# geopti/mjlab-1

Hardware: AMD Instinct MI355X
Metric: env-steps/sec, Unitree-G1 velocity task num_envs=4096, 1/2/4/8 MI355X (higher is better)
Workload: dtype f32

## Files before the change

mjlab-1_amd/csrc/engine_impl.h:

```cpp
#pragma once
#include <float.h>
#include <stdlib.h>
#include <algorithm>
#include <initializer_list>
#include <utility>
#include <math.h>

#include "engine.h"

#pragma clang fp contract(on)

namespace mjx {

#define MINVAL 1e-15f
#define MINMU 1e-5f
#define MINIMP 0.0001f
#define MAXIMP 0.9999f


struct V3 { float x, y, z; };
__device__ __forceinline__ V3 v3(const float* p) { return {p[0], p[1], p[2]}; }
__device__ __forceinline__ void st3(float* p, V3 a) { p[0] = a.x; p[1] = a.y; p[2] = a.z; }
__device__ __forceinline__ V3 operator+(V3 a, V3 b) { return {a.x + b.x, a.y + b.y, a.z + b.z}; }
__device__ __forceinline__ V3 operator-(V3 a, V3 b) { return {a.x - b.x, a.y - b.y, a.z - b.z}; }
// ... 2059 lines not shown
      spd_factor_solve_tree<NR, SP>(S + L.M, S + L.H, S + L.qacc_smooth, S + L.chol, nvp, lane);
    else
      spd_factor_solve<NR>(S + L.M, nullptr, S + L.H, S + L.qacc_smooth, S + L.chol, nvp, lane);
    const float qacs_i = lane < nvq ? S[L.qacc_smooth + lane] : 0.f;
    if (lane < nvq) gw[LB.qacc_smooth + lane] = qacs_i;
    STAMP(7);
    if (obs) {
      float* mb = S + L.crb;
      if (bl) mb[B.b] = B.mass;
      sync();
      const V3 X = v3(S + L.subtree_com + 3 * B.b);
      const V3 vown = v3(S + L.stlin + 3 * B.b);
      V3 pv = {0.f, 0.f, 0.f}, hs = {0.f, 0.f, 0.f}, cx = {0.f, 0.f, 0.f}, mr = {0.f, 0.f, 0.f};
#pragma unroll 4
      for (int c = 0; c < nb; c++) {
        const bool in = (B.sub >> c) & 1ull;
        const float f = in ? mb[c] : 0.f, fh = in ? 1.f : 0.f;
        const V3 r = v3(S + L.xipos + 3 * c) - X;
        const V3 vc = v3(S + L.stlin + 3 * c);
        pv = pv + vc * f;
        hs = hs + v3(S + L.stang + 3 * c) * fh;
        cx = cx + cross(r, vc) * f;
        mr = mr + r * f;
      }
      sync();
      if (bl) {
        const float sm = stm;
        const V3 V = sm > MINVAL ? pv * (1.0f / sm) : vown;
        st3(S + L.stlin + 3 * B.b, V);
        st3(S + L.stang + 3 * B.b, hs + cx - cross(mr, V));
      }
      sync();
    }
    for (int s = lane; obs && s < d.nsensor; s += kWave) {
      if (m.sensor_type[s] != SENS_SUBTREEANGMOM) continue;
      float* out = D.sensordata + (size_t)w * d.nsensordata + m.sensor_adr[s];
      const int obj = m.sensor_objid[s];
      out[0] = S[L.stang + 3 * obj]; out[1] = S[L.stang + 3 * obj + 1]; out[2] = S[L.stang + 3 * obj + 2];
    }
    if (last) {
      const size_t wb = (size_t)w * nb;
      for (int i = lane; i < 3 * nb; i += kWave) {
        D.subtree_linvel[wb * 3 + i] = S[L.stlin + i];
        D.subtree_angmom[wb * 3 + i] = S[L.stang + i];
      }
    }
    sync();
    STAMP(8);
    if (lane == 0) { ints[0] = 0; ints[1] = 0; ints[2] = 0; ints[3] = 0; }
    {
      const float* gpos = MF(geom_pos);
      const float* gquat = MF(geom_quat);
      for (int sl = lane; sl < d.ngeom_lds; sl += kWave) {
        const int g = m.lds_geom[sl];
        int b = m.geom_bodyid[g];
        const Q4 qb = q4(S + L.xquat + 4 * b);
        st3(S + L.gxpos + 3 * sl, v3(S + L.xpos + 3 * b) + qrot(qb, v3(gpos + 3 * g)));
        qmat(S + L.gxmat + 9 * sl, qmul(qb, q4(gquat + 4 * g)));
      }
    }
    sync();
    {
      ConOut co{S, ints, &L, d.nconmax};
      const float* gsize = MF(geom_size);
      const float* grb = MF(geom_rbound);
      const float* gmargin = MF(geom_margin);
      const bool rec = m.pair_rec != nullptr && m.geom_rbound_ws == 0 && m.geom_margin_ws == 0;
      for (int p = lane; p < d.npair; p += kWave) {
        int g1, g2, t1, t2, l1, l2;
        float margin, cull;
        if (rec) {
          const int4 rc = reinterpret_cast<const int4*>(m.pair_rec)[p];
          g1 = rc.x & 0xffff; g2 = (int)((unsigned)rc.x >> 16);
          l1 = rc.y & 0xfff; l2 = (rc.y >> 12) & 0xfff;
          t1 = (rc.y >> 24) & 15; t2 = (int)((unsigned)rc.y >> 28);
          margin = __int_as_float(rc.z);
          cull = __int_as_float(rc.w);
        } else {
          g1 = m.pair_geom1[p]; g2 = m.pair_geom2[p];
          t1 = m.geom_type[g1]; t2 = m.geom_type[g2];
          l1 = m.geom_lds[g1]; l2 = m.geom_lds[g2];
          margin = fmaxf(gmargin[g1], gmargin[g2]);
          const float r1 = grb[g1], r2 = grb[g2];
          cull = (r1 > 0 && r2 > 0 && t1 != GEOM_HFIELD) ? r1 + r2 + margin : INFINITY;
        }
        V3 p1 = v3(S + L.gxpos + 3 * l1), p2 = v3(S + L.gxpos + 3 * l2);
        if (norm(p2 - p1) > cull) continue;
        const float* s1 = gsize + 3 * g1;
        const float* s2 = gsize + 3 * g2;
        int key = p * 8;
        if (t1 == GEOM_PLANE) {
          const float* Rp = S + L.gxmat + 9 * l1;
          V3 n = {Rp[2], Rp[5], Rp[8]};
          if (t2 == GEOM_SPHERE) {
            plane_sphere(co, key, g1, g2, p1, n, p2, s2[0], margin);
          } else if (t2 == GEOM_CAPSULE) {
            const float* R2 = S + L.gxmat + 9 * l2;
            V3 ax = {R2[2], R2[5], R2[8]};
            int k = key;
            k += plane_sphere(co, k, g1, g2, p1, n, p2 + ax * s2[1], s2[0], margin);
            plane_sphere(co, k, g1, g2, p1, n, p2 - ax * s2[1], s2[0], margin);
          } else if (t2 == GEOM_BOX) {
            float dist = dot(p2 - p1, n);
            const float* R2 = S + L.gxmat + 9 * l2;
            int cnt = 0;
            for (int i = 0; i < 8 && cnt < 4; i++) {
              V3 v = {(i & 1) ? s2[0] : -s2[0], (i & 2) ? s2[1] : -s2[1], (i & 4) ? s2[2] : -s2[2]};
              V3 corner = mulv(R2, v);
              float ld = dot(n, corner);
              if (dist + ld > margin || ld > 0) continue;
              append(co, key + cnt, g1, g2, dist + ld, corner + p2 - n * (0.5f * (dist + ld)), n);
              cnt++;
            }
          } else {
            atomicOr(&ints[3], 4);
          }
        } else if (t1 == GEOM_SPHERE && t2 == GEOM_SPHERE) {
          sphere_sphere(co, key, g1, g2, p1, s1[0], p2, s2[0], margin);
        } else if (t1 == GEOM_SPHERE && t2 == GEOM_CAPSULE) {
          const float* R2 = S + L.gxmat + 9 * l2;
          V3 ax = {R2[2], R2[5], R2[8]};
          V3 pa, pb;
          seg_seg(p1, p1, p2 + ax * s2[1], p2 - ax * s2[1], &pa, &pb);
          sphere_sphere(co, key, g1, g2, p1, s1[0], pb, s2[0], margin);
        } else if (t1 == GEOM_CAPSULE && t2 == GEOM_CAPSULE) {
          const float* R1 = S + L.gxmat + 9 * l1;
          const float* R2 = S + L.gxmat + 9 * l2;
          const V3 a1 = {R1[2], R1[5], R1[8]}, a2 = {R2[2], R2[5], R2[8]};
          capsule_capsule(co, key, g1, g2, p1, a1 * s1[1], s1[0], p2, a2 * s2[1], s2[0], margin);
        } else if (t1 == GEOM_BOX && t2 == GEOM_BOX) {
          HFrame F1, F2;
          F1.p = p1; F2.p = p2;
          for (int i = 0; i < 9; i++) { F1.R[i] = S[L.gxmat + 9 * l1 + i]; F2.R[i] = S[L.gxmat + 9 * l2 + i]; }
          if constexpr (kBoxBox<SP>) box_box(co, key, g1, g2, F1, v3(s1), F2, v3(s2), margin);
        } else if (t2 == GEOM_BOX && (t1 == GEOM_SPHERE || t1 == GEOM_CAPSULE)) {
          HFrame F;
          F.p = p2;
#pragma unroll
          for (int i = 0; i < 9; i++) F.R[i] = S[L.gxmat + 9 * l2 + i];
          if (t1 == GEOM_SPHERE) {
            box_sphere(co, key, g1, g2, F, v3(s2), mulTv(F.R, p1 - F.p), s1[0], margin);
          } else {
            const float* R1 = S + L.gxmat + 9 * l1;
            box_capsule(co, key, g1, g2, F, v3(s2), p1, V3{R1[2], R1[5], R1[8]}, s1[1], s1[0], margin);
          }
        } else {
          atomicOr(&ints[3], 4);
        }
      }
      if (d.nstatic > 0) {
        float lo0 = 1e30f, lo1 = 1e30f, lo2 = 1e30f, hi0 = -1e30f, hi1 = -1e30f, hi2 = -1e30f;
        for (int i = lane; i < d.nstpartner; i += kWave) {
          const int g = m.st_partner[i];
          const V3 c = v3(S + L.gxpos + 3 * m.geom_lds[g]);
          const float r = grb[g] + gmargin[g];
          lo0 = fminf(lo0, c.x - r); lo1 = fminf(lo1, c.y - r); lo2 = fminf(lo2, c.z - r);
          hi0 = fmaxf(hi0, c.x + r); hi1 = fmaxf(hi1, c.y + r); hi2 = fmaxf(hi2, c.z + r);
        }
        lo0 = wave_min(lo0); lo1 = wave_min(lo1); lo2 = wave_min(lo2);
        hi0 = wave_max(hi0); hi1 = wave_max(hi1); hi2 = wave_max(hi2);
        auto overlap = [&](const float* bb) {
          return bb[0] <= hi0 && bb[3] >= lo0 && bb[1] <= hi1 && bb[4] >= lo1 && bb[2] <= hi2 &&
                 bb[5] >= lo2;
        };
        const float* gpos = MF(geom_pos);
        const float* gquat = MF(geom_quat);
        const float* hsz_all = MF(hfield_size);
        const float* hdat_all = MF(hfield_data);
        int trunc = 0;
        static_assert(kStaticChunk == kWave, "lane per terrain geom of a chunk");
        const int nchunk = (d.nstatic + kStaticChunk - 1) / kStaticChunk;
        for (int cb = 0; cb < nchunk; cb += kWave) {
          const int c = cb + lane;
          unsigned long long cbal = __ballot(c < nchunk && overlap(m.st_chunk_aabb + 6 * c));
          while (cbal) {
            const int ch = cb + __ffsll((long long)cbal) - 1;
            cbal &= cbal - 1;
            const int i = ch * kStaticChunk + lane;
            unsigned long long bal = __ballot(i < d.nstatic && overlap(m.st_aabb + 6 * i));
            while (bal) {
              const int j = ch * kStaticChunk + __ffsll((long long)bal) - 1;
              bal &= bal - 1;
              const int sg = m.st_geom[j];
              const HFrame F = hfield_frame(m, S, L, gpos, gquat, sg);
              if (m.geom_type[sg] == GEOM_HFIELD) {
                const int hid = m.geom_dataid[sg];
                const float* hs = hsz_all + 4 * hid;
                const float* hd = hdat_all + m.hfield_adr[hid];
                const int nr = m.hfield_nrow[hid], nc = m.hfield_ncol[hid];
                for (int p = m.st_pairadr[j] + lane; p < m.st_pairadr[j + 1]; p += kWave) {
                  const int g2 = m.pair_geom2[p];
                  const int t2 = m.geom_type[g2];
                  const int l2 = m.geom_lds[g2];
                  const V3 p2 = v3(S + L.gxpos + 3 * l2);
                  const float* s2 = gsize + 3 * g2;
                  const float margin = fmaxf(gmargin[sg], gmargin[g2]);
                  const int key = p * 8;
                  if (t2 == GEOM_SPHERE) {
                    hfield_sphere(co, key, sg, g2, F, hd, hs, nr, nc, p2, s2[0], margin, &trunc);
                  } else if (t2 == GEOM_CAPSULE) {
                    const float* R2 = S + L.gxmat + 9 * l2;
                    const V3 ax = {R2[2], R2[5], R2[8]};
                    int k = key;
                    k += hfield_sphere(co, k, sg, g2, F, hd, hs, nr, nc, p2 + ax * s2[1], s2[0], margin, &trunc);
                    hfield_sphere(co, k, sg, g2, F, hd, hs, nr, nc, p2 - ax * s2[1], s2[0], margin, &trunc);
                  } else {
                    atomicOr(&ints[3], 4);
                  }
                }
              } else {
                const float* bb = m.st_aabb + 6 * j;
                const V3 bs = v3(gsize + 3 * sg);
                for (int p = m.st_pairadr[j] + lane; p < m.st_pairadr[j + 1]; p += kWave) {
                  const int pa = m.pair_geom1[p], pb = m.pair_geom2[p];
                  const int g1 = pa == sg ? pb : pa;
                  const int t1 = m.geom_type[g1];
                  const int l1 = m.geom_lds[g1];
                  const V3 p1 = v3(S + L.gxpos + 3 * l1);
                  const float margin = fmaxf(gmargin[sg], gmargin[g1]);
                  const float rr = grb[g1] + margin;
                  if (p1.x + rr < bb[0] || p1.x - rr > bb[3] || p1.y + rr < bb[1] ||
                      p1.y - rr > bb[4] || p1.z + rr < bb[2] || p1.z - rr > bb[5]) continue;
                  const float* s1 = gsize + 3 * g1;
                  const int key = p * 8;
                  if (t1 == GEOM_SPHERE) {
                    box_sphere(co, key, g1, sg, F, bs, mulTv(F.R, p1 - F.p), s1[0], margin);
                  } else if (t1 == GEOM_CAPSULE) {
                    const float* R1 = S + L.gxmat + 9 * l1;
                    box_capsule(co, key, g1, sg, F, bs, p1, V3{R1[2], R1[5], R1[8]}, s1[1], s1[0], margin);
                  } else if (t1 == GEOM_BOX) {
                    HFrame Fp;
                    Fp.p = p1;
                    for (int i = 0; i < 9; i++) Fp.R[i] = S[L.gxmat + 9 * l1 + i];
                    if constexpr (kBoxBox<SP>) {
                      if (pa == sg) box_box(co, key, pa, pb, F, bs, Fp, v3(s1), margin);
                      else box_box(co, key, pa, pb, Fp, v3(s1), F, bs, margin);
                    }
                  } else {
                    atomicOr(&ints[3], 4);
                  }
                }
              }
            }
          }
        }
        if (trunc) atomicOr(&ints[3], 4);
      }
    }
    sync();
    STAMP(3);
    int ncon = min(ints[0], d.nconmax);
    {
      auto contact_params = [&](int c, int g1, int g2, float dist) {
        const float* fri = MF(geom_friction);
        const float* sref = MF(geom_solref);
        const float* simp = MF(geom_solimp);
        const float* smix = MF(geom_solmix);
        const float* gmar = MF(geom_margin);
        const float* ggap = MF(geom_gap);
        int p1 = m.geom_priority[g1], p2 = m.geom_priority[g2];
        int dim;
        float f0, f1;
        float sr[2], si[5];
        if (p1 != p2) {
          int g = p1 > p2 ? g1 : g2;
          dim = m.geom_condim[g];
          f0 = fri[3 * g]; f1 = fri[3 * g + 1];
          sr[0] = sref[2 * g]; sr[1] = sref[2 * g + 1];
          for (int i = 0; i < 5; i++) si[i] = simp[5 * g + i];
        } else {
          dim = max(m.geom_condim[g1], m.geom_condim[g2]);
          f0 = fmaxf(fri[3 * g1], fri[3 * g2]);
          f1 = fmaxf(fri[3 * g1 + 1], fri[3 * g2 + 1]);
          float s1 = smix[g1], s2 = smix[g2], mix;
          if (s1 < MINVAL && s2 < MINVAL) mix = 0.5f;
          else if (s1 < MINVAL) mix = 0.f;
          else if (s2 < MINVAL) mix = 1.f;
          else mix = s1 / (s1 + s2);
          const float* r1 = sref + 2 * g1;
          const float* r2 = sref + 2 * g2;
          if (r1[0] > 0 && r2[0] > 0) {
            sr[0] = mix * r1[0] + (1 - mix) * r2[0];
            sr[1] = mix * r1[1] + (1 - mix) * r2[1];
          } else {
            sr[0] = fminf(r1[0], r2[0]);
            sr[1] = fminf(r1[1], r2[1]);
          }
          for (int i = 0; i < 5; i++) si[i] = mix * simp[5 * g1 + i] + (1 - mix) * simp[5 * g2 + i];
        }
        (void)f1;
        S[L.con_mu + 2 * c] = fmaxf(MINMU, f0);
        S[L.con_mu + 2 * c + 1] = fmaxf(MINMU, f0);
        Si[L.con_dim + c] = dim;
        const float imargin = fmaxf(gmar[g1], gmar[g2]) - fmaxf(ggap[g1], ggap[g2]);
        S[L.con_imargin + c] = imargin;
        S[L.con_imp + c] = impedance(si, dist, imargin);
        solref_kb(sr, si, h, S[L.con_kb + 2 * c], S[L.con_kb + 2 * c + 1]);
      };
      auto con_bodies = [&](int g1, int g2) {
        const int b1 = m.geom_bodyid[g1], b2 = m.geom_bodyid[g2];
        return b1 | b2 << 8 | m.body_rootid[b1] << 16 | m.body_rootid[b2] << 24;
      };
      if (kCon1<SP> || ncon <= kWave) {
        int key = lane < ncon ? Si[L.con_key + lane] : 0x7fffffff;
        int idx = lane;
#pragma unroll
        for (int k = 2; k <= kWave; k <<= 1) {
#pragma unroll
          for (int j = k >> 1; j > 0; j >>= 1) {
            int pk = __shfl_xor(key, j);
            int pi = __shfl_xor(idx, j);
            bool up = (lane & k) == 0;
            bool lower = (lane & j) == 0;
            bool sw = lower ? (up ? key > pk : key < pk) : (up ? key < pk : key > pk);
            if (sw) { key = pk; idx = pi; }
          }
        }
        int g1 = 0, g2 = 0;
        float dist = 0, px = 0, py = 0, pz = 0, nx = 0, ny = 0, nz = 0;
        if (lane < ncon) {
          g1 = Si[L.con_g1 + idx]; g2 = Si[L.con_g2 + idx]; dist = S[L.con_dist + idx];
          px = S[L.con_pos + 3 * idx]; py = S[L.con_pos + 3 * idx + 1]; pz = S[L.con_pos + 3 * idx + 2];
          nx = S[L.con_n + 3 * idx]; ny = S[L.con_n + 3 * idx + 1]; nz = S[L.con_n + 3 * idx + 2];
        }
        sync();
        if (lane < ncon) {
          Si[L.con_g1 + lane] = g1; Si[L.con_g2 + lane] = g2; S[L.con_dist + lane] = dist;
          Si[L.con_key + lane] = con_bodies(g1, g2);
          S[L.con_pos + 3 * lane] = px; S[L.con_pos + 3 * lane + 1] = py; S[L.con_pos + 3 * lane + 2] = pz;
          V3 n = {nx, ny, nz};
          n = n * (1.0f / fmaxf(norm(n), MINVAL));
          st3(S + L.con_n + 3 * lane, n);
          contact_params(lane, g1, g2, dist);
        }
      } else if constexpr (!kCon1<SP>) {
        int* perm = Si + L.efc_cid;
        const int rounds = (ncon + kWave - 1) / kWave;
        for (int c = lane; c < ncon; c += kWave) {
          const int kc = Si[L.con_key + c];
          int rank = 0;
          for (int j = 0; j < ncon; j++) rank += Si[L.con_key + j] < kc ? 1 : 0;
          perm[rank] = c;
        }
        sync();
        auto permute = [&](float* base, int stride, int comp) {
          float v[kMaxConRounds];
#pragma unroll
          for (int r = 0; r < kMaxConRounds; r++) {
            const int c = lane + r * kWave;
            v[r] = r < rounds && c < ncon ? base[stride * perm[c] + comp] : 0.f;
          }
          sync();
#pragma unroll
          for (int r = 0; r < kMaxConRounds; r++) {
            const int c = lane + r * kWave;
            if (r < rounds && c < ncon) base[stride * c + comp] = v[r];
          }
          sync();
        };
        permute(reinterpret_cast<float*>(Si + L.con_g1), 1, 0);
        permute(reinterpret_cast<float*>(Si + L.con_g2), 1, 0);
        permute(S + L.con_dist, 1, 0);
        for (int t = 0; t < 3; t++) permute(S + L.con_pos, 3, t);
        for (int t = 0; t < 3; t++) permute(S + L.con_n, 3, t);
        for (int c = lane; c < ncon; c += kWave) {
          const int g1 = Si[L.con_g1 + c], g2 = Si[L.con_g2 + c];
          Si[L.con_key + c] = con_bodies(g1, g2);
          V3 n = v3(S + L.con_n + 3 * c);
          n = n * (1.0f / fmaxf(norm(n), MINVAL));
          st3(S + L.con_n + 3 * c, n);
          contact_params(c, g1, g2, S[L.con_dist + c]);
        }
      }
      sync();
    }
    STAMP(4);
    {
      const float* jrange = MF(jnt_range);
      const float* jmargin = MF(jnt_margin);
      int nlim_rows = 0;
      int lim_mask = 0;
      if (lane < d.njnt && m.jnt_limited[lane] &&
          (m.jnt_type[lane] == JNT_HINGE || m.jnt_type[lane] == JNT_SLIDE)) {
        float q = S[L.qpos + m.jnt_qposadr[lane]];
        float mg = jmargin[lane];
        if (q - jrange[2 * lane] < mg) lim_mask |= 1;
        if (jrange[2 * lane + 1] - q < mg) lim_mask |= 2;
        nlim_rows = (lim_mask & 1) + ((lim_mask >> 1) & 1);
      }
      int lim_total, lim_off = wave_excl_scan(nlim_rows, lane, &lim_total);
      const bool con1 = kCon1<SP> || ncon <= kWave;
      int cdim = 0, crow = 0, con_total = 0, con_off = 0;
      if (con1) {
        cdim = lane < ncon ? Si[L.con_dim + lane] : 0;
        crow = lane < ncon ? (cdim == 1 ? 1 : 2 * (cdim - 1)) : 0;
        if (lane < ncon && cdim != 1 && cdim != 3) atomicOr(&ints[3], 4);
        con_off = wave_excl_scan(crow, lane, &con_total);
      } else {
        for (int c0 = 0; c0 < ncon; c0 += kWave) {
          const int c = c0 + lane;
          const int cd = c < ncon ? Si[L.con_dim + c] : 0;
          const int cr = c < ncon ? (cd == 1 ? 1 : 2 * (cd - 1)) : 0;
          if (c < ncon && cd != 1 && cd != 3) atomicOr(&ints[3], 4);
          int tot, off = wave_excl_scan(cr, lane, &tot);
          if (c < ncon) Si[L.con_efc + c] = con_total + off;
          con_total += tot;
        }
      }
      auto con_rows = [&](int c) {
        const int cd = Si[L.con_dim + c];
        return cd == 1 ? 1 : 2 * (cd - 1);
      };
      int nefc = lim_total + con_total;
      if (P->ovf_resolve) {
        const bool over = ints[0] > d.nconmax || nefc > d.njmax;
        int slot = -1;
        if (over && lane == 0) {
          const int li = 2 * split + ((sel_arg & kSelAPar) ? 1 : 0);
          slot = atomicAdd(P->ovf_n + li, 1);
          if (slot < P->ovf_cap) {
            P->ovf_list[(size_t)li * P->ovf_cap + slot] = w;
            atomicAdd(D.evtotal + 3, 1);
          }
        }
        slot = __shfl(slot, 0);
        const bool listed = over && slot < P->ovf_cap;
        if (lane == 0) {
          P->ovf_flag[w] = listed ? 1 : 0;
          if (listed) D.nefc[w] = -1;
        }
        if (listed) return;
      }
      if (nefc > d.njmax) {
        if (lane == 0) atomicOr(&ints[3], 2);
      }
      int keep_con = ncon;
      if (con1) {
        bool fits = lane < ncon && lim_total + con_off + crow <= d.njmax;
        unsigned long long bal = __ballot(lane < ncon && !fits);
        if (bal) keep_con = __ffsll((long long)bal) - 1;
        keep_con = min(keep_con, ncon);
        ncon = keep_con;
        nefc = lim_total + (ncon > 0 ? __shfl(con_off + crow, ncon - 1) : 0);
      } else {
        for (int c0 = 0; c0 < ncon; c0 += kWave) {
          const int c = c0 + lane;
          const bool fits = c < ncon && lim_total + Si[L.con_efc + c] + con_rows(c) <= d.njmax;
          const unsigned long long bal = __ballot(c < ncon && !fits);
          if (bal) { keep_con = c0 + __ffsll((long long)bal) - 1; break; }
        }
        ncon = keep_con;
        nefc = lim_total + (ncon > 0 ? Si[L.con_efc + ncon - 1] + con_rows(ncon - 1) : 0);
      }
      if (lim_total > d.njmax) { nefc = 0; ncon = 0; }
      const float* dinvw = MF(dof_invweight0);
      const float* binvw = MF(body_invweight0);
      const float* jsolref = MF(jnt_solref);
      const float* jsolimp = MF(jnt_solimp);
      if (lim_mask && nefc > 0) {
        int r = lim_off;
        float q = S[L.qpos + m.jnt_qposadr[lane]];
        for (int side = -1; side <= 1; side += 2) {
          if (!((side < 0 ? lim_mask & 1 : lim_mask & 2))) continue;
          float dist = side * (jrange[2 * lane + (side + 1) / 2] - q);
          Si[L.efc_cid + r] = efc_code(EFC_LIMIT, lane | m.jnt_dofadr[lane] << 8);
          S[L.efc_aref + r] = dist;
          S[L.efc_D + r] = (float)(-side);
          r++;
        }
      }
      bool xbranch = false;
      if constexpr (kTree<SP>) {
        for (int c = lane; c < ncon; c += kWave) {
          const int cbk = Si[L.con_key + c];
          const uint64_t m1 = m.body_dofmask[cb_b1(cbk)], m2 = m.body_dofmask[cb_b2(cbk)];
          xbranch |= (m1 & ~m2) != 0ull && (m2 & ~m1) != 0ull;
        }
      }
      const int dense_h = __ballot(xbranch) != 0ull || !kTree<SP>;
      if (con1) {
        if (lane < ncon) {
          int r0 = lim_total + con_off;
          Si[L.con_efc + lane] = r0;
          for (int k = 0; k < crow; k++)
            Si[L.efc_cid + r0 + k] = efc_code(cdim == 1 ? EFC_FRICTIONLESS : EFC_PYRAMIDAL, lane);
        }
      } else {
        for (int c = lane; c < ncon; c += kWave) {
          const int r0 = lim_total + Si[L.con_efc + c];
          const int cd = Si[L.con_dim + c];
          Si[L.con_efc + c] = r0;
          for (int k = 0; k < con_rows(c); k++)
            Si[L.efc_cid + r0 + k] = efc_code(cd == 1 ? EFC_FRICTIONLESS : EFC_PYRAMIDAL, c);
        }
      }
      sync();
      const int ngrp = nvp <= kWave / 2 ? kWave / nvp : 1;
      const int grp = lane / nvp;
      for (int i = lane - grp * nvp; grp < ngrp && i < nvp; i += kWave) {
        for (int r = grp; r < lim_total && r < nefc; r += ngrp) {
          const int jd = Si[L.efc_cid + r] >> 2;
          Jg[r * nvp + i] = (jd >> 8) == i ? S[L.efc_D + r] : 0.f;
        }
        if (i >= nv) {
          for (int r = lim_total + grp; r < nefc; r += ngrp) Jg[r * nvp + i] = 0.f;
          continue;
        }
        uint64_t bm = m.dof_bodymask[i];
        const float* cd = S + L.cdof + 6 * i;
        V3 cang = v3(cd), clin = v3(cd + 3);
        for (int c = grp; c < ncon; c += ngrp) {
          const int cb = Si[L.con_key + c];
          const int b1 = cb_b1(cb), b2 = cb_b2(cb);
          V3 pos = v3(S + L.con_pos + 3 * c);
          V3 jd = {0, 0, 0};
          if (b2 > 0 && ((bm >> b2) & 1ull))
            jd = jd + clin + cross(cang, pos - v3(S + L.subtree_com + 3 * cb_r2(cb)));
          if (b1 > 0 && ((bm >> b1) & 1ull))
            jd = jd - (clin + cross(cang, pos - v3(S + L.subtree_com + 3 * cb_r1(cb))));
          const CFrame F = cframe(v3(S + L.con_n + 3 * c));
          float jn = dot(F.n, jd);
          int r0 = Si[L.con_efc + c];
          if (Si[L.con_dim + c] == 1) {
            Jg[r0 * nvp + i] = jn;
          } else {
            float jt1 = dot(F.t, jd);
            float jt2 = dot(F.b, jd);
            float mu0 = S[L.con_mu + 2 * c], mu1 = S[L.con_mu + 2 * c + 1];
            Jg[(r0 + 0) * nvp + i] = jn + mu0 * jt1;
            Jg[(r0 + 1) * nvp + i] = jn - mu0 * jt1;
            Jg[(r0 + 2) * nvp + i] = jn + mu1 * jt2;
            Jg[(r0 + 3) * nvp + i] = jn - mu1 * jt2;
          }
        }
      }
      sync();
      for (int r = lane; r < nefc; r += kWave) {
        const int code = Si[L.efc_cid + r];
        const int type = code & 3, pl = code >> 2;
        float pos, margin, diag, imp, K, B;
        if (type == EFC_LIMIT) {
          const int j = pl & 255;
          pos = S[L.efc_aref + r];
          margin = jmargin[j];
          diag = dinvw[pl >> 8];
          imp = impedance(jsolimp + 5 * j, pos, margin);
          solref_kb(jsolref + 2 * j, jsolimp + 5 * j, h, K, B);
        } else {
          const int c = pl;
          pos = S[L.con_dist + c];
          margin = S[L.con_imargin + c];
          const int cb = Si[L.con_key + c];
          float tran = binvw[2 * cb_b1(cb)] + binvw[2 * cb_b2(cb)];
          if (type == EFC_FRICTIONLESS) {
            diag = tran;
          } else {
            float mu = S[L.con_mu + 2 * c + ((r - Si[L.con_efc + c]) >> 1)];
            diag = (tran + mu * mu * tran) / o.impratio;
          }
          imp = S[L.con_imp + c];
          K = S[L.con_kb + 2 * c];
          B = S[L.con_kb + 2 * c + 1];
        }
        float Rr = fmaxf(MINVAL, (1 - imp) * diag / imp);
        float vel;
        if (type == EFC_LIMIT) {
          vel = S[L.efc_D + r] * S[L.qvel + (pl >> 8)];
        } else {
          const int c = pl;
          V3 pc = v3(S + L.con_pos + 3 * c);
          const int cb = Si[L.con_key + c];
          V3 v = point_vel_r(S, L, cb_b2(cb), cb_r2(cb), pc) - point_vel_r(S, L, cb_b1(cb), cb_r1(cb), pc);
          const CFrame F = cframe(v3(S + L.con_n + 3 * c));
          vel = dot(F.n, v);
          if (type != EFC_FRICTIONLESS) {
            int kr = r - Si[L.con_efc + c];
            const V3 t = (kr >> 1) ? F.b : F.t;
            float mu = S[L.con_mu + 2 * c + (kr >> 1)];
            vel += ((kr & 1) ? -mu : mu) * dot(t, v);
          }
        }
        S[L.efc_D + r] = 1.0f / Rr;
        S[L.efc_aref + r] = -B * vel - K * imp * (pos - margin);
      }
      if (lane == 0) { ints[1] = nefc; ints[2] = lim_total; ints[4] = ncon; ints[6] = dense_h; }
      sync();
    }
    const int nefc = ints[1];
    ncon = ints[4];
    if (lane == 0) D.nefc[w] = nefc;
    STAMP(5);
    for (int s = lane; obs && s < d.nsensor; s += kWave) {
      float* out = D.sensordata + (size_t)w * d.nsensordata + m.sensor_adr[s];
      int obj = m.sensor_objid[s];
      int type = m.sensor_type[s];
      if ((type == SENS_ACCELEROMETER || type == SENS_CONTACT) != (PH == 2)) continue;
      if (type == SENS_CONTACT && m.sensor_intprm[3 * s + 2] <= 1 && m.ncsens > 0 &&
          (kCon1<SP> || ncon <= kWave)) continue;
      if (type == SENS_GYRO || type == SENS_VELOCIMETER || type == SENS_ACCELEROMETER) {
        int b = m.site_bodyid[obj];
        const float* R = S + L.sxmat + 9 * obj;
        const float* cv = S + L.cvel + 6 * b;
        V3 rel = v3(S + L.sxpos + 3 * obj) - v3(S + L.subtree_com + 3 * m.body_rootid[b]);
        V3 r;
        if (type == SENS_GYRO) {
          r = mulTv(R, v3(cv));
        } else {
          V3 v = v3(cv + 3) + cross(v3(cv), rel);
          if (type == SENS_VELOCIMETER) {
            r = mulTv(R, v);
          } else {
            const float* ca = S + L.cacc + 6 * b;
            V3 a = v3(ca + 3) + cross(v3(ca), rel) + cross(v3(cv), v);
            r = mulTv(R, a);
          }
        }
        out[0] = r.x; out[1] = r.y; out[2] = r.z;
      } else if (type == SENS_SUBTREEANGMOM) {
      } else if (type == SENS_FRAMEPOS) {
        const float* p = m.sensor_objtype[s] == OBJ_SITE ? S + L.sxpos + 3 * obj : S + L.xpos + 3 * obj;
        out[0] = p[0]; out[1] = p[1]; out[2] = p[2];
      } else if (type == SENS_JOINTPOS) {
        out[0] = S[L.qpos + m.jnt_qposadr[obj]];
      } else if (type == SENS_JOINTVEL) {
        out[0] = S[L.qvel + m.jnt_dofadr[obj]];
      } else if (type == SENS_CONTACT) {
        const int32_t* ip = m.sensor_intprm + 3 * s;
        int bits = ip[0], reduce = ip[1], nslot = min(ip[2], 8);
        const uint32_t* mk1 = m.sensor_geommask1 + m.nmaskword * s;
        const uint32_t* mk2 = m.sensor_geommask2 + m.nmaskword * s;
        int fdim = ((bits & 1) || (bits & 8)) ? 1 : 3;
        int dim = m.sensor_dim[s];
        for (int i = 0; i < dim; i++) out[i] = 0.f;
        int found = 0;
        V3 net = {0, 0, 0};
        int sel[8];
        float key[8];
        int nsel = 0;
        for (int c = 0; c < ncon; c++) {
          int g1 = Si[L.con_g1 + c], g2 = Si[L.con_g2 + c];
          bool a1 = ((mk1[g1 >> 5] >> (g1 & 31)) & 1u) && ((mk2[g2 >> 5] >> (g2 & 31)) & 1u);
          bool a2 = ((mk1[g2 >> 5] >> (g2 & 31)) & 1u) && ((mk2[g1 >> 5] >> (g1 & 31)) & 1u);
          if (!a1 && !a2) continue;
          if (found >= o.maxmatch) continue;
          found++;
          int r0 = Si[L.con_efc + c];
          V3 f = {0, 0, 0};
          if (Si[L.con_dim + c] == 1) {
            f.x = S[L.efc_force + r0];
          } else {
            float e0 = S[L.efc_force + r0], e1 = S[L.efc_force + r0 + 1];
            float e2 = S[L.efc_force + r0 + 2], e3 = S[L.efc_force + r0 + 3];
            f = {e0 + e1 + e2 + e3, (e0 - e1) * S[L.con_mu + 2 * c], (e2 - e3) * S[L.con_mu + 2 * c + 1]};
          }
          V3 fg = frame_tv(S + L.con_n + 3 * c, f);
          net = net + fg * (a1 ? 1.f : -1.f);
          float k = reduce == REDUCE_MINDIST ? S[L.con_dist + c]
                  : reduce == REDUCE_MAXFORCE ? -norm(f) : (float)nsel;
          if (nsel < nslot || k < key[nsel - 1]) {
            int pos = nsel < nslot ? nsel++ : nslot - 1;
            while (pos > 0 && key[pos - 1] > k) { key[pos] = key[pos - 1]; sel[pos] = sel[pos - 1]; pos--; }
            key[pos] = k;
            sel[pos] = c * 2 + (a1 ? 0 : 1);
          }
        }
        if (reduce == REDUCE_NETFORCE) {
          if (bits & 1) out[0] = (float)found;
          else if (bits & 2) { out[0] = net.x; out[1] = net.y; out[2] = net.z; }
        } else {
          for (int k = 0; k < nsel; k++) {
            int c = sel[k] >> 1;
            float sg = (sel[k] & 1) ? -1.f : 1.f;
            float* oo = out + k * fdim;
            if (bits & 1) oo[0] = (float)found;
            else if (bits & 8) oo[0] = S[L.con_dist + c];
            else if (bits & 16) { for (int t = 0; t < 3; t++) oo[t] = S[L.con_pos + 3 * c + t]; }
            else if (bits & 32) { for (int t = 0; t < 3; t++) oo[t] = sg * S[L.con_n + 3 * c + t]; }
            else if (bits & 64) { for (int t = 0; t < 3; t++) oo[t] = sg * vc(cframe(v3(S + L.con_n + 3 * c)).t, t); }
            else if (bits & 2) {
              int r0 = Si[L.con_efc + c];
              if (Si[L.con_dim + c] == 1) { oo[0] = S[L.efc_force + r0]; oo[1] = oo[2] = 0; }
              else {
                float e0 = S[L.efc_force + r0], e1 = S[L.efc_force + r0 + 1];
                float e2 = S[L.efc_force + r0 + 2], e3 = S[L.efc_force + r0 + 3];
                oo[0] = e0 + e1 + e2 + e3;
                oo[1] = (e0 - e1) * S[L.con_mu + 2 * c];
                oo[2] = (e2 - e3) * S[L.con_mu + 2 * c + 1];
              }
            }
          }
        }
      }
    }
    STAMP(11);
#ifdef MJX_ABLATE_OUTPUTS
    if (false) {
#else
    if (last) {
#endif
      size_t wb = (size_t)w * nb;
      for (int i = lane; i < 3 * nb; i += kWave) {
        D.xpos[wb * 3 + i] = S[L.xpos + i];
        D.xipos[wb * 3 + i] = S[L.xipos + i];
        D.subtree_com[wb * 3 + i] = S[L.subtree_com + i];
      }
      for (int i = lane; i < 4 * nb; i += kWave) D.xquat[wb * 4 + i] = S[L.xquat + i];
      if (bl) {
        float R[9], Ri[9];
        qmat(R, xq);
        qmat(Ri, qmul(xq, B.iquat));
        float* om = D.xmat + (wb + B.b) * 9;
        float* oi = D.ximat + (wb + B.b) * 9;
#pragma unroll
        for (int t = 0; t < 9; t++) { om[t] = R[t]; oi[t] = Ri[t]; }
      }
      for (int i = lane; i < 6 * nb; i += kWave) D.cvel[wb * 6 + i] = S[L.cvel + i];
      size_t wg = (size_t)w * d.ngeom;
      for (int i = lane; i < d.ngeom_lds; i += kWave) {
        const size_t g = wg + m.lds_geom[i];
        const float* xp = S + L.gxpos + 3 * i;
        const float* xm = S + L.gxmat + 9 * i;
        float* op = D.geom_xpos + g * 3;
        float* om = D.geom_xmat + g * 9;
#pragma unroll
        for (int t = 0; t < 3; t++) op[t] = xp[t];
#pragma unroll
        for (int t = 0; t < 9; t++) om[t] = xm[t];
      }
      size_t ws = (size_t)w * d.nsite;
      for (int i = lane; i < 3 * d.nsite; i += kWave) D.site_xpos[ws * 3 + i] = S[L.sxpos + i];
      for (int i = lane; i < 9 * d.nsite; i += kWave) D.site_xmat[ws * 9 + i] = S[L.sxmat + i];
      for (int i = lane; i < nv; i += kWave) {
        size_t k = (size_t)w * nv + i;
        D.qacc_smooth[k] = qacs_i;
        D.qfrc_bias[k] = qbias_i;
        D.qfrc_passive[k] = qpass_i;
        D.qfrc_actuator[k] = qact_i;
        D.qfrc_smooth[k] = qfs_i;
      }
      if (lane < nu) D.actuator_force[(size_t)w * nu + lane] = act_f;
      size_t wc = (size_t)w * P->con_stride;
      int* wsv = D.wstats + 8 * (size_t)w;
      const int nout = min(P->con_stride, max(ncon, wsv[7]));
      for (int c = lane; c < nout; c += kWave) {
        bool v = c < ncon;
        D.contact_dist[wc + c] = v ? S[L.con_dist + c] : 0.f;
        D.contact_geom[(wc + c) * 2] = v ? Si[L.con_g1 + c] : -1;
        D.contact_geom[(wc + c) * 2 + 1] = v ? Si[L.con_g2 + c] : -1;
        for (int t = 0; t < 3; t++) D.contact_pos[(wc + c) * 3 + t] = v ? S[L.con_pos + 3 * c + t] : 0.f;
        const CFrame F = cframe(v ? v3(S + L.con_n + 3 * c) : V3{0.f, 0.f, 1.f});
        const float fr[9] = {F.n.x, F.n.y, F.n.z, F.t.x, F.t.y, F.t.z, F.b.x, F.b.y, F.b.z};
        for (int t = 0; t < 9; t++) D.contact_frame[(wc + c) * 9 + t] = v ? fr[t] : 0.f;
      }
      if (lane == 0) { D.ncon[w] = ncon; D.nefc[w] = nefc; wsv[6] = nout; wsv[7] = ncon; }
    }
    STAMP(12);
    const int C = ncon;
    const int C4 = (C + 3) & ~3;
    const int nr4 = (nefc + 3) & ~3;
    cp4(gw + LB.ints, S + L.ints, 8, lane);
    cp4(gw + LB.efc_aref, S + L.efc_aref, nr4, lane);
    cp4(gw + LB.efc_D, S + L.efc_D, nr4, lane);
    if (obs) {
      cp4(gc + LC.cdof, S + L.cdof, 6 * nvp, lane);
      cp4(gc + LC.cvel, S + L.cvel, (6 * nb + 3) & ~3, lane);
      cp4(gc + LC.subtree_com, S + L.subtree_com, (3 * nb + 3) & ~3, lane);
    }
    if (obs) {
      cp4(gc + LC.sxpos, S + L.sxpos, (3 * d.nsite + 3) & ~3, lane);
      cp4(gc + LC.sxmat, S + L.sxmat, (9 * d.nsite + 3) & ~3, lane);
    }
    cp4(gc + LC.con_g1, S + L.con_g1, C4, lane);
    cp4(gc + LC.con_g2, S + L.con_g2, C4, lane);
    if (obs) {
      cp4(gc + LC.con_dist, S + L.con_dist, C4, lane);
      cp4(gc + LC.con_pos, S + L.con_pos, (3 * C + 3) & ~3, lane);
      cp4(gc + LC.con_n, S + L.con_n, (3 * C + 3) & ~3, lane);
      cp4(gc + LC.con_mu, S + L.con_mu, (2 * C + 3) & ~3, lane);
      cp4(gc + LC.con_dim, S + L.con_dim, C4, lane);
      cp4(gc + LC.con_efc, S + L.con_efc, C4, lane);
    }
    STAMP(14);
  } else if constexpr (PH == 1) {
    {
      const int nefc_in = reinterpret_cast<const int*>(gw)[LB.ints + 1];
      const int cls = integrate;
      cp_pack(S, gw, L.M + ltr_size(nvp), lane);
      if (JG) {
        cp_pack(S + L.qacc_smooth, gw + LB.qacc_smooth, LB.efc_J - LB.qacc_smooth, lane);
      } else if (cls <= 0) {
        cp_pack(S + L.qacc_smooth, gw + L.qacc_smooth, L.efc_J + nefc_in * nvp - L.qacc_smooth, lane);
      } else {
        const int nr4 = (nefc_in + 3) & ~3;
        cp_pack(S + L.qacc_smooth, gw + LB.qacc_smooth, LB.efc_aref + nr4 - LB.qacc_smooth, lane);
        cp_pack(S + L.efc_D, gw + LB.efc_D, nr4, lane);
        cp_pack(S + L.efc_J, gw + LB.efc_J, nefc_in * nvp, lane);
      }
    }
    const Tiles T = make_tiles(nvp, lane);
    for (int i = lane; i < nvp; i += kWave) {
      S[L.x + i] = 0.f; S[L.Mx + i] = 0.f;
      S[L.srch + i] = 0.f; S[L.Ms + i] = 0.f; S[L.qfrc_con + i] = 0.f;
      S[L.qacc_ws + i] = i < nv ? D.qacc_warmstart[(size_t)w * nv + i] : 0.f;
    }
    lds_dma_wait();
    sync();
    const int nefc = ints[1];
    int ncon = ints[4];
    (void)ncon;
    const bool tree_h = kTree<SP> && !MJX_JTDJ_MFMA && __builtin_amdgcn_readfirstlane(ints[6]) == 0;
    float Mt[2][16];
    tiles_load_ltr(Mt, T, S + L.M);
    sync();
    STAMP(15);
    int niter = 0;
    if (nefc == 0) {
      for (int i = lane; i < nvp; i += kWave) {
        S[L.x + i] = S[L.qacc_smooth + i];
        S[L.qfrc_con + i] = 0.f;
      }
      sync();
    } else {
      float* jar = S + L.efc_jar;
      float* Js = S + L.efc_Js;
      float* wv = S + L.efc_force;
      const float* Dv = S + L.efc_D;
      const float* J = JG ? gw + LB.efc_J : S + L.efc_J;
      int* act = Si + L.efc_act;
      float* Lm = S + L.H;
      const float scale = 1.0f / (o.meaninertia * (float)max(nv, 1));
#ifdef MJX_STAMPS
      sub_prev = __builtin_amdgcn_s_memtime();
      stamp_acc[38] += 1;
      stamp_acc[39] += !tree_h;
#endif
      const bool reg_rows = nefc <= kWave;
// ... 723 lines not shown
```

Measured before the change: 3.029 million.

## Replace bitonic contact sort with readlane rank scatter and broadcast contact data

The in-wave bitonic sort of contact keys becomes a rank count per lane using readlane over the other lanes' keys, followed by scattering each contact into its sorted slot. This removes the gather by permuted index. For the single-group Jacobian case, each lane now loads one contact's frame, position and COM data once, and the data is broadcast to all DOF lanes with readlane. This replaces having every lane re-read the contact data from shared memory. The risk is a serial loop over ncon, and ties in equal keys could collide in the rank scatter.

Result: faster. 3.075 million, median of 6 (+1.5%).

```diff
diff --git a/mjlab-1_amd/csrc/engine_impl.h b/mjlab-1_amd/csrc/engine_impl.h
--- a/mjlab-1_amd/csrc/engine_impl.h
+++ b/mjlab-1_amd/csrc/engine_impl.h
@@ -2385,36 +2385,29 @@
         return b1 | b2 << 8 | m.body_rootid[b1] << 16 | m.body_rootid[b2] << 24;
       };
       if (kCon1<SP> || ncon <= kWave) {
-        int key = lane < ncon ? Si[L.con_key + lane] : 0x7fffffff;
-        int idx = lane;
-#pragma unroll
-        for (int k = 2; k <= kWave; k <<= 1) {
-#pragma unroll
-          for (int j = k >> 1; j > 0; j >>= 1) {
-            int pk = __shfl_xor(key, j);
-            int pi = __shfl_xor(idx, j);
-            bool up = (lane & k) == 0;
-            bool lower = (lane & j) == 0;
-            bool sw = lower ? (up ? key > pk : key < pk) : (up ? key < pk : key > pk);
-            if (sw) { key = pk; idx = pi; }
-          }
+        const int nc = __builtin_amdgcn_readfirstlane(ncon);
+        int pos = lane;
+        if (nc > 1) {
+          const int key = lane < nc ? Si[L.con_key + lane] : 0x7fffffff;
+          pos = 0;
+          for (int j = 0; j < nc; j++) pos += __builtin_amdgcn_readlane(key, j) < key ? 1 : 0;
         }
         int g1 = 0, g2 = 0;
         float dist = 0, px = 0, py = 0, pz = 0, nx = 0, ny = 0, nz = 0;
         if (lane < ncon) {
-          g1 = Si[L.con_g1 + idx]; g2 = Si[L.con_g2 + idx]; dist = S[L.con_dist + idx];
-          px = S[L.con_pos + 3 * idx]; py = S[L.con_pos + 3 * idx + 1]; pz = S[L.con_pos + 3 * idx + 2];
-          nx = S[L.con_n + 3 * idx]; ny = S[L.con_n + 3 * idx + 1]; nz = S[L.con_n + 3 * idx + 2];
+          g1 = Si[L.con_g1 + lane]; g2 = Si[L.con_g2 + lane]; dist = S[L.con_dist + lane];
+          px = S[L.con_pos + 3 * lane]; py = S[L.con_pos + 3 * lane + 1]; pz = S[L.con_pos + 3 * lane + 2];
+          nx = S[L.con_n + 3 * lane]; ny = S[L.con_n + 3 * lane + 1]; nz = S[L.con_n + 3 * lane + 2];
         }
         sync();
         if (lane < ncon) {
-          Si[L.con_g1 + lane] = g1; Si[L.con_g2 + lane] = g2; S[L.con_dist + lane] = dist;
-          Si[L.con_key + lane] = con_bodies(g1, g2);
-          S[L.con_pos + 3 * lane] = px; S[L.con_pos + 3 * lane + 1] = py; S[L.con_pos + 3 * lane + 2] = pz;
+          Si[L.con_g1 + pos] = g1; Si[L.con_g2 + pos] = g2; S[L.con_dist + pos] = dist;
+          Si[L.con_key + pos] = con_bodies(g1, g2);
+          S[L.con_pos + 3 * pos] = px; S[L.con_pos + 3 * pos + 1] = py; S[L.con_pos + 3 * pos + 2] = pz;
           V3 n = {nx, ny, nz};
           n = n * (1.0f / fmaxf(norm(n), MINVAL));
-          st3(S + L.con_n + 3 * lane, n);
-          contact_params(lane, g1, g2, dist);
+          st3(S + L.con_n + 3 * pos, n);
+          contact_params(pos, g1, g2, dist);
         }
       } else if constexpr (!kCon1<SP>) {
         int* perm = Si + L.efc_cid;
@@ -2580,6 +2573,66 @@
       sync();
       const int ngrp = nvp <= kWave / 2 ? kWave / nvp : 1;
       const int grp = lane / nvp;
+      auto con_jrows = [&](int i, uint64_t bm, V3 cang, V3 clin, int cb, V3 pos, V3 com1, V3 com2,
+                           const CFrame& F, int dim, int r0, float mu0, float mu1) {
+        const int b1 = cb_b1(cb), b2 = cb_b2(cb);
+        V3 jd = {0, 0, 0};
+        if (b2 > 0 && ((bm >> b2) & 1ull)) jd = jd + clin + cross(cang, pos - com2);
+        if (b1 > 0 && ((bm >> b1) & 1ull)) jd = jd - (clin + cross(cang, pos - com1));
+        float jn = dot(F.n, jd);
+        if (dim == 1) {
+          Jg[r0 * nvp + i] = jn;
+        } else {
+          float jt1 = dot(F.t, jd);
+          float jt2 = dot(F.b, jd);
+          Jg[(r0 + 0) * nvp + i] = jn + mu0 * jt1;
+          Jg[(r0 + 1) * nvp + i] = jn - mu0 * jt1;
+          Jg[(r0 + 2) * nvp + i] = jn + mu1 * jt2;
+          Jg[(r0 + 3) * nvp + i] = jn - mu1 * jt2;
+        }
+      };
+      if (con1 && ngrp == 1 && nvp <= kWave) {
+        const int i = lane;
+        int kcb = 0, kdim = 0, kr0 = 0;
+        float kmu0 = 0, kmu1 = 0;
+        V3 kpos = {0, 0, 0}, kc1 = {0, 0, 0}, kc2 = {0, 0, 0};
+        CFrame kF = {{0, 0, 0}, {0, 0, 0}, {0, 0, 0}};
+        if (lane < ncon) {
+          kcb = Si[L.con_key + lane];
+          kdim = cdim;
+          kr0 = lim_total + con_off;
+          kmu0 = S[L.con_mu + 2 * lane]; kmu1 = S[L.con_mu + 2 * lane + 1];
+          kpos = v3(S + L.con_pos + 3 * lane);
+          kF = cframe(v3(S + L.con_n + 3 * lane));
+          kc1 = v3(S + L.subtree_com + 3 * cb_r1(kcb));
+          kc2 = v3(S + L.subtree_com + 3 * cb_r2(kcb));
+        }
+        uint64_t bm = 0;
+        V3 cang = {0, 0, 0}, clin = {0, 0, 0};
+        if (i < nvp) {
+          for (int r = 0; r < lim_total && r < nefc; r++) {
+            const int jd = Si[L.efc_cid + r] >> 2;
+            Jg[r * nvp + i] = (jd >> 8) == i ? S[L.efc_D + r] : 0.f;
+          }
+          if (i >= nv) {
+            for (int r = lim_total; r < nefc; r++) Jg[r * nvp + i] = 0.f;
+          } else {
+            bm = m.dof_bodymask[i];
+            const float* cd = S + L.cdof + 6 * i;
+            cang = v3(cd); clin = v3(cd + 3);
+          }
+        }
+        const auto rli = [](int v, int l) { return __builtin_amdgcn_readlane(v, l); };
+        const auto rl3 = [](V3 v, int l) { return V3{rl(v.x, l), rl(v.y, l), rl(v.z, l)}; };
+        const int nc = __builtin_amdgcn_readfirstlane(ncon);
+        for (int c = 0; c < nc; c++) {
+          const int cb = rli(kcb, c), dim = rli(kdim, c), r0 = rli(kr0, c);
+          const float mu0 = rl(kmu0, c), mu1 = rl(kmu1, c);
+          const V3 pos = rl3(kpos, c), com1 = rl3(kc1, c), com2 = rl3(kc2, c);
+          const CFrame F = {rl3(kF.n, c), rl3(kF.t, c), rl3(kF.b, c)};
+          if (i < nv) con_jrows(i, bm, cang, clin, cb, pos, com1, com2, F, dim, r0, mu0, mu1);
+        }
+      } else
       for (int i = lane - grp * nvp; grp < ngrp && i < nvp; i += kWave) {
         for (int r = grp; r < lim_total && r < nefc; r += ngrp) {
           const int jd = Si[L.efc_cid + r] >> 2;
@@ -2594,27 +2647,10 @@
         V3 cang = v3(cd), clin = v3(cd + 3);
         for (int c = grp; c < ncon; c += ngrp) {
           const int cb = Si[L.con_key + c];
-          const int b1 = cb_b1(cb), b2 = cb_b2(cb);
-          V3 pos = v3(S + L.con_pos + 3 * c);
-          V3 jd = {0, 0, 0};
-          if (b2 > 0 && ((bm >> b2) & 1ull))
-            jd = jd + clin + cross(cang, pos - v3(S + L.subtree_com + 3 * cb_r2(cb)));
-          if (b1 > 0 && ((bm >> b1) & 1ull))
-            jd = jd - (clin + cross(cang, pos - v3(S + L.subtree_com + 3 * cb_r1(cb))));
-          const CFrame F = cframe(v3(S + L.con_n + 3 * c));
-          float jn = dot(F.n, jd);
-          int r0 = Si[L.con_efc + c];
-          if (Si[L.con_dim + c] == 1) {
-            Jg[r0 * nvp + i] = jn;
-          } else {
-            float jt1 = dot(F.t, jd);
-            float jt2 = dot(F.b, jd);
-            float mu0 = S[L.con_mu + 2 * c], mu1 = S[L.con_mu + 2 * c + 1];
-            Jg[(r0 + 0) * nvp + i] = jn + mu0 * jt1;
-            Jg[(r0 + 1) * nvp + i] = jn - mu0 * jt1;
-            Jg[(r0 + 2) * nvp + i] = jn + mu1 * jt2;
-            Jg[(r0 + 3) * nvp + i] = jn - mu1 * jt2;
-          }
+          con_jrows(i, bm, cang, clin, cb, v3(S + L.con_pos + 3 * c),
+                    v3(S + L.subtree_com + 3 * cb_r1(cb)), v3(S + L.subtree_com + 3 * cb_r2(cb)),
+                    cframe(v3(S + L.con_n + 3 * c)), Si[L.con_dim + c], Si[L.con_efc + c],
+                    S[L.con_mu + 2 * c], S[L.con_mu + 2 * c + 1]);
         }
       }
       sync();
```
